# sglang-npu/DeepGEMM_Ascend

Measured on AMD Instinct MI355X. Metric: fp8 TFLOPS + % MFMA peak, 4096^3 block-scaled GEMM; grouped-GEMM tok/s at 1/2/4/8 GPU, higher is better.
Workload: dtype bf16

## Files before the change

deepgemm_ascend_amd/csrc/dga_launch_menu_n.hip:

```cpp
#include <atomic>
#include <cstdlib>
#include "dga_fp8_menu_impl.hpp"
#include "gemm_fp8_bf16x_dsk_kernel.hpp"
namespace dga {

static constexpr int kDskExtraHalfBlocks = 2;

int bx_dsk_splits(int64_t tiles, int kb, int want, int cus)
{
    if (tiles <= 0 || tiles > cus) return 0;
    int s = want > 0 ? want : 1;
    if (s > DskCfg::MAX_S) s = DskCfg::MAX_S;
    if (s > cus / tiles) s = static_cast<int>(cus / tiles);
    if (s > kb / 4) s = kb / 4;
    return s;
}

size_t bx_dsk_workspace_bytes(int64_t tiles, int splits)
{
    if (splits <= 1) return 0;
    return static_cast<size_t>(tiles) * (splits - 1) * (DskCfg::SLOT_FLOATS * 4 + 8) + 256;
}

template <bool KTAIL, bool IMG = true, int OUT = 0>
static int launch_bx_dsk_one(const GemmParams &p, const StreamKArgs &sk, unsigned grid, hipStream_t stream)
{
    constexpr int kLds = IMG ? DskCfg::IMG_LDS_BYTES : DskCfg::LDS_BYTES;
    return launch_kernel<gemm_fp8_bf16x_dsk_kernel<KTAIL, IMG, OUT>>(grid, DskCfg::NT, kLds, stream, p, sk);
}

int launch_bf16x_dsk(const GemmParams &p, int splits, void *ws, size_t ws_bytes, hipStream_t stream, Out out)
{
    if (out == Out::F32Rows) return DGA_E_TILING;
    if (p.groups != 1 || p.masked_m || p.m_indices || p.row_index || p.splitk > 1 || p.tail_sub || p.stamps || p.launch_tiles) return DGA_E_TILING;
    const int cus = coresident_workgroups(stream);
    if (cus <= 0) return DGA_E_TILING;
    GemmParams q = p;
    q.tiles_m = (p.m + DskCfg::BM - 1) / DskCfg::BM;
    q.tiles_n = (p.n + DskCfg::BN - 1) / DskCfg::BN;
    const int64_t tiles = static_cast<int64_t>(q.tiles_m) * q.tiles_n;
    const int s = bx_dsk_splits(tiles, p.kb_n, splits, cus);
    if (s < 1) return DGA_E_TILING;
    q.splitk = s;
    StreamKArgs sk{};
    if (s > 1) {
        const size_t slots = static_cast<size_t>(tiles) * (s - 1);
        if (!ws || ws_bytes < slots * (DskCfg::SLOT_FLOATS * 4 + 8) || (reinterpret_cast<uintptr_t>(ws) & 15)) return DGA_E_TILING;
        sk.partials = static_cast<float *>(ws);
        sk.flags = reinterpret_cast<unsigned long long *>(sk.partials + slots * DskCfg::SLOT_FLOATS);
        static std::atomic<unsigned long long> launches{0};
        const unsigned long long e = launches.fetch_add(1) + 1;
        sk.epoch = (e * 0x9E3779B97F4A7C15ull) | 1ull;
    }
    if (s > 1) {
        int extra = kDskExtraHalfBlocks;
#ifdef DGA_DSK_KNOBS
        if (const char *e = std::getenv("DGA_DSK_EXTRA")) extra = std::atoi(e);
#endif
        for (; extra > 0; --extra) {
            const int wo = (2 * p.kb_n - 2 * extra) / (2 * s), wa = wo + extra;
            if (wo < 4 || wa > 255 || wo > 255) continue;
            const int64_t W = 2 * wa + static_cast<int64_t>(2 * s - 2) * wo;
            auto cut = [&](int i) { return static_cast<int>((static_cast<int64_t>(p.kb_n) * (i <= 2 ? i * wa : 2 * wa + (i - 2) * wo)) / W); };
            bool ok = true;
            for (int i = 0; i < 2 * s && ok; ++i) ok = cut(i + 1) - cut(i) >= 2;
            if (ok) { q.tail_sub = wa | (wo << 8); break; }
        }
    }
#ifdef DGA_DSK_KNOBS
    if (const char *e = std::getenv("DGA_DSK_KNOB")) q.tail_begin = std::atoi(e);
#endif
    const unsigned grid = static_cast<unsigned>(tiles * s);
#ifdef DGA_DSK_KNOBS
    if (q.tail_begin & 64)
        return (p.k % 128) ? launch_bx_dsk_one<true, false>(q, sk, grid, stream) : launch_bx_dsk_one<false, false>(q, sk, grid, stream);
#endif
    if (out == Out::F32) return (p.k % 128) ? launch_bx_dsk_one<true, true, 1>(q, sk, grid, stream) : launch_bx_dsk_one<false, true, 1>(q, sk, grid, stream);
    return (p.k % 128) ? launch_bx_dsk_one<true>(q, sk, grid, stream) : launch_bx_dsk_one<false>(q, sk, grid, stream);
}

}
```

deepgemm_ascend_amd/csrc/gemm_fp8_bf16x_dsk_kernel.hpp:

```cpp
#pragma once
#include "gemm_fp8_kernel.hpp"
#include "gemm_fp8_streamk_kernel.hpp"

namespace dga {

struct DskCfg {
    static constexpr int BM = 64, BN = 128, GT = 256, NT = 512, TN = 2;
    static constexpr int A_BYTES = BM * 128, B_BYTES = BN * 128, SC_BYTES = GT * 4;
    static constexpr int STAGE_BYTES = A_BYTES + B_BYTES + SC_BYTES, RING_BYTES = 3 * STAGE_BYTES, LDS_BYTES = 2 * RING_BYTES;
    static constexpr int IMG_BYTES = BM * 128 * 2, IMG_GROUP_BYTES = 2 * STAGE_BYTES + IMG_BYTES, IMG_LDS_BYTES = 2 * IMG_GROUP_BYTES;
    static constexpr int A_ITERS = 2, B_ITERS = 4, NL = A_ITERS + B_ITERS + 1;
    static constexpr int SLOT_FLOATS = BM * BN;
    static constexpr int MAX_S = 8;
};

template <bool KTAIL, bool IMG = true, int OUT = 0>
__global__ void __launch_bounds__(512) __attribute__((amdgpu_waves_per_eu(2, 2)))
gemm_fp8_bf16x_dsk_kernel(const GemmParams p, const StreamKArgs sk)
{
    typedef DskCfg C;
    constexpr int BM = C::BM, BN = C::BN, GT = C::GT, TN = C::TN, NL = C::NL, LAGT = 2, RING = 4;
    typedef __bf16 v8bf __attribute__((ext_vector_type(8)));
    extern __shared__ __attribute__((aligned(16))) uint8_t smem[];

    const int tid = threadIdx.x, lane = tid & 63, gtid = tid & (GT - 1);
    const int wave = __builtin_amdgcn_readfirstlane(tid >> 6);
    const int h = wave >> 2, gw = wave & 3;
    const int li = lane & 15, kg = lane >> 4;
    const int KB = p.kb_n, S = p.splitk;

    int v = blockIdx.x;
    if (p.xcd_remap) v = xcd_chunk_first(gridDim.x, v & 7) + (v >> 3);
    const int tm = v % p.tiles_m, rest = v / p.tiles_m, s = rest % S, tn = rest / S;
    const int tile = tn * p.tiles_m + tm;
    const int M = p.m, m0 = tm * BM, n0 = tn * BN;
    const int wa = p.tail_sub > 0 ? (p.tail_sub & 0xFF) : 1, wo = p.tail_sub > 0 ? (p.tail_sub >> 8) : 1;
    const int W = 2 * wa + (2 * S - 2) * wo;
    auto cut = [&](int i) { return (int)(((int64_t)KB * (i <= 2 ? i * wa : 2 * wa + (i - 2) * wo)) / W); };
    const int i0 = 2 * s + h, io = 2 * s + (1 - h);
    const int kb0 = cut(i0), kb1 = cut(i0 + 1);
    const int nblk = kb1 - kb0;
    const int nblk_o = cut(io + 1) - cut(io);
    const int nmax = max(nblk, nblk_o);

    uint8_t *const ring = smem + h * (IMG ? C::IMG_GROUP_BYTES : C::RING_BYTES);
    const uint32_t lds0 = (uint32_t)(uintptr_t)(lptr_t)ring;
    constexpr uint32_t kOutOfRange = 0x80000000u;
    const int a_col = ((gtid & 7) ^ swz_a(gtid >> 3)) * 16;
    const int b_col = ((gtid & 7) ^ swz_b(gtid >> 3)) * 16;
    uint32_t a_voff[C::A_ITERS], b_voff[C::B_ITERS];
#pragma unroll
    for (int it = 0; it < C::A_ITERS; ++it) {
        const int row = (it * GT + gtid) >> 3;
        a_voff[it] = row < M - m0 ? (uint32_t)row * (uint32_t)p.lda + a_col : kOutOfRange;
    }
#pragma unroll
    for (int it = 0; it < C::B_ITERS; ++it) {
        const int row = (it * GT + gtid) >> 3;
        b_voff[it] = (uint32_t)min(row, p.n - 1 - n0) * (uint32_t)p.ldb + b_col;
    }
    const v4i a_rsrc = make_rsrc(p.a + (int64_t)m0 * p.lda, (int64_t)(M - m0) * p.lda);
    const v4i b_rsrc = make_rsrc(p.b + (int64_t)n0 * p.ldb, (int64_t)(p.n - n0) * p.ldb);
    const float *const sc_src = gtid < BM ? p.sfa + (int64_t)min(m0 + gtid, M - 1) * p.sfa_ld
                                          : p.sfb + (int64_t)min(n0 / 128, p.nb_n - 1) * p.kb_n;
    auto refill = [&](int idx, int stage, int kb) {
#ifdef DGA_DSK_KNOBS
        if (p.tail_begin & 8) return;
#endif
        const uint32_t sa = lds0 + stage * C::STAGE_BYTES + gw * 1024;
        const int k0 = kb * 128;
        const bool live = kb < kb1;
        if (idx < C::A_ITERS) {
            uint32_t voff = live ? a_voff[idx] : kOutOfRange;
            if constexpr (KTAIL) voff = (k0 + a_col < p.k) ? voff : kOutOfRange;
            dma16(voff, a_rsrc, (uint32_t)k0, sa + idx * GT * 16);
        } else if (idx < C::A_ITERS + C::B_ITERS) {
            const int it = idx - C::A_ITERS;
            uint32_t voff = live ? b_voff[it] : kOutOfRange;
            if constexpr (KTAIL) voff = (k0 + b_col < p.k) ? voff : kOutOfRange;
            dma16(voff, b_rsrc, (uint32_t)k0, sa + C::A_BYTES + it * GT * 16);
        } else {
            dma4(sc_src + (live ? kb : kb1 - 1), lds0 + stage * C::STAGE_BYTES + C::A_BYTES + C::B_BYTES + gw * 256);
        }
    };

    const int a_off0 = li * 128 + ((kg ^ swz_a(li)) * 16);
    const int a_off1 = li * 128 + (((kg + 4) ^ swz_a(li)) * 16);
    const int b_row = gw * (BN / 4) + 8 * (li >> 2) + (li & 3);
    const int b_off0 = C::A_BYTES + b_row * 128 + ((kg ^ swz_b(b_row)) * 16);
    const int b_off1 = C::A_BYTES + b_row * 128 + (((kg + 4) ^ swz_b(b_row)) * 16);
    const int sa_off = C::A_BYTES + C::B_BYTES + li * 4;
    const int sb_off = C::A_BYTES + C::B_BYTES + BM * 4;

    v4f acc[4][TN];
    v4f part[RING];
    v4i afx[2][4], bfx[TN][4];
    v4i braw[TN][2], araw[2][2];
    float s_cur[4], s_old[4];
#pragma unroll
    for (int i = 0; i < 4; ++i)
#pragma unroll
        for (int j = 0; j < TN; ++j) acc[i][j] = v4f{0.f, 0.f, 0.f, 0.f};

#pragma unroll
    for (int d = 0; d < (IMG ? 2 : 3); ++d)
#pragma unroll
        for (int idx = 0; idx < NL; ++idx) refill(idx, d, kb0 + d);

    auto run = [&](auto Lc) __attribute__((always_inline)) {
        constexpr int L = decltype(Lc)::value;
        constexpr int TILES = L * TN, GAPS = 4 * TILES, SP = L;
        static_assert(TILES % RING == 0 && 1 + (NL - 1) * SP < GAPS, "the ring of partial tiles; the refill fits a block");
#pragma unroll
        for (int i = 0; i < RING; ++i) part[i] = v4f{0.f, 0.f, 0.f, 0.f};
#pragma unroll
        for (int i = 0; i < L; ++i) s_old[i] = 0.f;
        int cur = 0;
        for (int it = 0; it < nmax; ++it) {
            if (it == 0) wait_vmcnt<2 * NL>();
            else wait_vmcnt<NL>();
            __builtin_amdgcn_s_barrier();
            asm volatile("" ::: "memory");
#ifdef DGA_DSK_KNOBS
            if ((p.tail_begin & 4) && it < nblk) {
                if (it > 0) for (int idx = 0; idx < NL; ++idx) refill(idx, cur >= 1 ? cur - 1 : 2, kb0 + it + 2);
            } else
#endif
            if (it < nblk) {
                const int fill = cur >= 1 ? cur - 1 : 2, kbf = kb0 + it + 2;
                const uint8_t *sc = ring + cur * C::STAGE_BYTES;
#ifdef DGA_DSK_KNOBS
                if ((p.tail_begin & 32) && it > 0)
                    for (int idx = 0; idx < NL; ++idx) refill(idx, fill, kbf);
#endif
                araw[0][0] = *(const v4i *)(sc + a_off0);
                araw[0][1] = *(const v4i *)(sc + a_off1);
                braw[0][0] = *(const v4i *)(sc + b_off0);
                braw[0][1] = *(const v4i *)(sc + b_off1);
                braw[1][0] = *(const v4i *)(sc + b_off0 + 512);
                braw[1][1] = *(const v4i *)(sc + b_off1 + 512);
                araw[1][0] = *(const v4i *)(sc + a_off0 + 2048);
                araw[1][1] = *(const v4i *)(sc + a_off1 + 2048);
                const float sfb0 = *(const float *)(sc + sb_off);
                float sa[L];
#pragma unroll
                for (int i = 0; i < L; ++i) sa[i] = *(const float *)(sc + sa_off + i * 64);
                __builtin_amdgcn_sched_barrier(0);
#pragma unroll
                for (int c = 0; c < 16; ++c) bx_convert(braw[0], bfx[0], c);
#pragma unroll
                for (int c = 0; c < 16; ++c) bx_convert(araw[0], afx[0], c);
                if constexpr (L > 2) {
                    araw[0][0] = *(const v4i *)(sc + a_off0 + 2 * 2048);
                    araw[0][1] = *(const v4i *)(sc + a_off1 + 2 * 2048);
                }
#pragma unroll
                for (int c = 0; c < 16; ++c) bx_convert(braw[1], bfx[1], c);
#pragma unroll
                for (int i = 0; i < L; ++i) s_cur[i] = sa[i] * sfb0;
                __builtin_amdgcn_sched_barrier(0);
#pragma unroll
                for (int u = 0; u < GAPS; ++u) {
                    const int t = u >> 2, q = u & 3, mt = t / TN, nt = t % TN, g8 = u % (4 * TN);
                    part[t % RING] = __builtin_amdgcn_mfma_f32_16x16x32_bf16(
                        __builtin_bit_cast(v8bf, bfx[nt][q]), __builtin_bit_cast(v8bf, afx[mt & 1][q]),
                        q == 0 ? v4f{0.f, 0.f, 0.f, 0.f} : part[t % RING], 0, 0, 0);
                    __builtin_amdgcn_sched_barrier(0);
#ifdef DGA_DSK_KNOBS
                    if (!(p.tail_begin & 32))
#endif
                    if (u >= 1 && (u - 1) % SP == 0 && (u - 1) / SP < NL && it > 0) refill((u - 1) / SP, fill, kbf);
                    if (mt + 1 < L) {
#pragma unroll
                        for (int c = 2 * g8; c < 2 * g8 + 2; ++c) bx_convert(araw[(mt + 1) & 1], afx[(mt + 1) & 1], c);
                        if (g8 == 4 * TN - 1 && mt + 3 < L) {
                            araw[(mt + 1) & 1][0] = *(const v4i *)(sc + a_off0 + (mt + 3) * 2048);
                            araw[(mt + 1) & 1][1] = *(const v4i *)(sc + a_off1 + (mt + 3) * 2048);
                        }
                    }
                    {
                        const int j = t >= LAGT ? t - LAGT : TILES + t - LAGT, jm = j / TN, jn = j % TN;
                        const float sv = t >= LAGT ? s_cur[jm] : s_old[jm];
                        acc[jm][jn][q] = __builtin_fmaf(part[j % RING][q], sv, acc[jm][jn][q]);
                    }
                    __builtin_amdgcn_sched_barrier(0);
                }
#pragma unroll
                for (int i = 0; i < L; ++i) s_old[i] = s_cur[i];
            }
            cur = cur == 2 ? 0 : cur + 1;
        }
#pragma unroll
        for (int t = 0; t < LAGT; ++t) {
            const int j = TILES + t - LAGT, jm = j / TN, jn = j % TN;
#pragma unroll
            for (int q = 0; q < 4; ++q) acc[jm][jn][q] = __builtin_fmaf(part[j % RING][q], s_old[jm], acc[jm][jn][q]);
        }
    };
    auto run_img = [&](auto Lc) __attribute__((always_inline)) {
        constexpr int L = decltype(Lc)::value;
        constexpr int TILES = L * TN, GAPS = 4 * TILES, SP = L;
        static_assert(TILES % RING == 0 && 1 + (NL - 1) * SP < GAPS, "the ring of partial tiles; the refill fits a block");
        uint8_t *const img = ring + 2 * C::STAGE_BYTES;
#pragma unroll
        for (int i = 0; i < RING; ++i) part[i] = v4f{0.f, 0.f, 0.f, 0.f};
#pragma unroll
        for (int i = 0; i < L; ++i) s_old[i] = 0.f;
        int cur = 0;
        for (int it = 0; it < nmax; ++it) {
            wait_vmcnt<NL>();
            __builtin_amdgcn_s_barrier();
            asm volatile("" ::: "memory");
            const bool live = it < nblk;
            const uint8_t *sc = ring + cur * C::STAGE_BYTES;
            if (live) {
                if (gw < L) {
                    araw[0][0] = *(const v4i *)(sc + a_off0 + gw * 2048);
                    araw[0][1] = *(const v4i *)(sc + a_off1 + gw * 2048);
                }
                braw[0][0] = *(const v4i *)(sc + b_off0);
                braw[0][1] = *(const v4i *)(sc + b_off1);
                braw[1][0] = *(const v4i *)(sc + b_off0 + 512);
                braw[1][1] = *(const v4i *)(sc + b_off1 + 512);
                const float sfb0 = *(const float *)(sc + sb_off);
                float sa[L];
#pragma unroll
                for (int i = 0; i < L; ++i) sa[i] = *(const float *)(sc + sa_off + i * 64);
                if (gw < L) {
#pragma unroll
                    for (int c = 0; c < 16; ++c) bx_convert(araw[0], afx[0], c);
#pragma unroll
                    for (int q = 0; q < 4; ++q) *(v4i *)(img + ((gw * 4 + q) * 64 + lane) * 16) = afx[0][q];
                }
#pragma unroll
                for (int c = 0; c < 16; ++c) bx_convert(braw[0], bfx[0], c);
#pragma unroll
                for (int c = 0; c < 16; ++c) bx_convert(braw[1], bfx[1], c);
#pragma unroll
                for (int i = 0; i < L; ++i) s_cur[i] = sa[i] * sfb0;
            }
            asm volatile("s_waitcnt lgkmcnt(0)" ::: "memory");
            __builtin_amdgcn_s_barrier();
            asm volatile("" ::: "memory");
            if (live) {
                const int kbf = kb0 + it + 2;
#pragma unroll
                for (int q = 0; q < 4; ++q) afx[0][q] = *(const v4i *)(img + (q * 64 + lane) * 16);
                __builtin_amdgcn_sched_barrier(0);
#pragma unroll
                for (int u = 0; u < GAPS; ++u) {
                    const int t = u >> 2, q = u & 3, mt = t / TN, nt = t % TN;
                    part[t % RING] = __builtin_amdgcn_mfma_f32_16x16x32_bf16(
                        __builtin_bit_cast(v8bf, bfx[nt][q]), __builtin_bit_cast(v8bf, afx[mt & 1][q]),
                        q == 0 ? v4f{0.f, 0.f, 0.f, 0.f} : part[t % RING], 0, 0, 0);
                    __builtin_amdgcn_sched_barrier(0);
                    if (u >= 1 && (u - 1) % SP == 0 && (u - 1) / SP < NL) refill((u - 1) / SP, cur, kbf);
                    if (nt == 0 && q == 0 && mt + 1 < L) {
#pragma unroll
                        for (int qq = 0; qq < 4; ++qq) afx[(mt + 1) & 1][qq] = *(const v4i *)(img + (((mt + 1) * 4 + qq) * 64 + lane) * 16);
                    }
                    {
                        const int j = t >= LAGT ? t - LAGT : TILES + t - LAGT, jm = j / TN, jn = j % TN;
                        const float sv = t >= LAGT ? s_cur[jm] : s_old[jm];
                        acc[jm][jn][q] = __builtin_fmaf(part[j % RING][q], sv, acc[jm][jn][q]);
                    }
                    __builtin_amdgcn_sched_barrier(0);
                }
#pragma unroll
                for (int i = 0; i < L; ++i) s_old[i] = s_cur[i];
            }
            cur ^= 1;
        }
#pragma unroll
        for (int t = 0; t < LAGT; ++t) {
            const int j = TILES + t - LAGT, jm = j / TN, jn = j % TN;
#pragma unroll
            for (int q = 0; q < 4; ++q) acc[jm][jn][q] = __builtin_fmaf(part[j % RING][q], s_old[jm], acc[jm][jn][q]);
        }
    };
    if constexpr (IMG) {
        if (M - m0 <= 32) run_img(std::integral_constant<int, 2>{});
        else run_img(std::integral_constant<int, 4>{});
    } else {
        if (M - m0 <= 32) run(std::integral_constant<int, 2>{});
        else run(std::integral_constant<int, 4>{});
    }

    wait_vmcnt<0>();
    __builtin_amdgcn_s_barrier();
    asm volatile("" ::: "memory");
    v4f *const X = reinterpret_cast<v4f *>(smem);
    if (h == 1) {
#pragma unroll
        for (int ti = 0; ti < 8; ++ti) X[(gw * 8 + ti) * 64 + lane] = acc[ti >> 1][ti & 1];
    }
    __syncthreads();
    if (h == 0) {
#pragma unroll
        for (int ti = 0; ti < 8; ++ti) {
            const v4f o = X[(gw * 8 + ti) * 64 + lane];
            v4f &a = acc[ti >> 1][ti & 1];
            a.x += o.x; a.y += o.y; a.z += o.z; a.w += o.w;
        }
    }
    uint16_t *const Cout = p.out;
    const bool vec_ok = ((p.ldc & 7) == 0) && ((((uintptr_t)Cout) & 15) == 0);
    auto store_row = [&](int m, int n, const v4f &lo, const v4f &hi) {
        if (m >= M) return;
        if constexpr (OUT == 1) {
            float *const Cf = reinterpret_cast<float *>(p.out);
            const v4f v[2] = {lo, hi};
            store_row_f32<8>(Cf + (int64_t)m * p.ldc, p.c_in ? p.c_in + (int64_t)m * p.ldc : nullptr, n, p.n,
                             f32_rows_vec(Cf, p.c_in, p.ldc), 0, v);
            return;
        }
        uint16_t *crow = Cout + (int64_t)m * p.ldc;
        const v2bf h0 = __builtin_convertvector(v2f{lo.x, lo.y}, v2bf);
        const v2bf h1 = __builtin_convertvector(v2f{lo.z, lo.w}, v2bf);
        const v2bf h2 = __builtin_convertvector(v2f{hi.x, hi.y}, v2bf);
        const v2bf h3 = __builtin_convertvector(v2f{hi.z, hi.w}, v2bf);
        const v4i pk = v4i{__builtin_bit_cast(int, h0), __builtin_bit_cast(int, h1), __builtin_bit_cast(int, h2), __builtin_bit_cast(int, h3)};
        if (vec_ok && n + 8 <= p.n) {
            *(v4i *)(crow + n) = pk;
        } else {
            const uint16_t *e = (const uint16_t *)&pk;
#pragma unroll
            for (int q = 0; q < 8; ++q)
                if (n + q < p.n) crow[n + q] = e[q];
        }
    };
    if (S == 1) {
        if (h == 0) {
#pragma unroll
            for (int mt = 0; mt < 4; ++mt) store_row(m0 + 16 * mt + li, n0 + gw * (BN / 4) + 8 * kg, acc[mt][0], acc[mt][1]);
        }
        return;
    }
#ifdef DGA_DSK_KNOBS
    const int knob = p.tail_begin;
    if ((knob & 1) && s > 0) return;
#endif
    if (s > 0) {
        const int slot = tile * (S - 1) + (s - 1);
        if (h == 0) {
            float *dst = sk.partials + (int64_t)slot * C::SLOT_FLOATS + (gw * 8 * 64 + lane) * 4;
#pragma unroll
            for (int ti = 0; ti < 8; ++ti) {
                asm volatile("global_store_dwordx4 %0, %1, off sc0 sc1" :: "v"(dst), "v"(acc[ti >> 1][ti & 1]) : "memory");
                dst += 64 * 4;
                asm volatile("" : "+v"(dst));
            }
        }
        wait_vmcnt<0>();
        __builtin_amdgcn_s_barrier();
        asm volatile("" ::: "memory");
        if (tid == 0) __hip_atomic_store(sk.flags + slot, sk.epoch, __ATOMIC_RELAXED, __HIP_MEMORY_SCOPE_AGENT);
        return;
    }
    if (h == 0) {
#pragma unroll
        for (int ti = 0; ti < 8; ++ti) X[(gw * 8 + ti) * 64 + lane] = acc[ti >> 1][ti & 1];
    }
    const int e0 = (gw * 8 + 4 * h) * 64 + lane;
    v4f w[C::MAX_S - 1][4];
    __syncthreads();
#pragma unroll
    for (int j = 0; j < C::MAX_S - 1; ++j) {
        if (j < S - 1) {
#ifdef DGA_DSK_KNOBS
            if (!(knob & 3))
#endif
            if (tid == 0)
                while (__hip_atomic_load(sk.flags + tile * (S - 1) + j, __ATOMIC_RELAXED, __HIP_MEMORY_SCOPE_AGENT) != sk.epoch) __builtin_amdgcn_s_sleep(2);
            __builtin_amdgcn_s_barrier();
            asm volatile("" ::: "memory");
            if (wave != 0) {
                const float *src = sk.partials + (int64_t)(tile * (S - 1) + j) * C::SLOT_FLOATS + e0 * 4;
#pragma unroll
                for (int e = 0; e < 4; ++e) {
                    asm volatile("global_load_dwordx4 %0, %1, off sc0 sc1" : "=v"(w[j][e]) : "v"(src) : "memory");
                    src += 64 * 4;
                    asm volatile("" : "+v"(src));
                }
            }
        }
    }
    if (wave == 0) {
#pragma unroll
        for (int j = 0; j < C::MAX_S - 1; ++j) {
            if (j < S - 1) {
                const float *src = sk.partials + (int64_t)(tile * (S - 1) + j) * C::SLOT_FLOATS + e0 * 4;
#pragma unroll
                for (int e = 0; e < 4; ++e) {
                    asm volatile("global_load_dwordx4 %0, %1, off sc0 sc1" : "=v"(w[j][e]) : "v"(src) : "memory");
                    src += 64 * 4;
                    asm volatile("" : "+v"(src));
                }
            }
        }
    }
    if (tid == 0)
        for (int j = 0; j < S - 1; ++j) __hip_atomic_store(sk.flags + tile * (S - 1) + j, 0ull, __ATOMIC_RELAXED, __HIP_MEMORY_SCOPE_AGENT);
    v4f sum[4];
#pragma unroll
    for (int e = 0; e < 4; ++e) sum[e] = X[e0 + 64 * e];
    wait_vmcnt<0>();
#pragma unroll
    for (int j = 0; j < C::MAX_S - 1; ++j) {
        if (j < S - 1) {
#pragma unroll
            for (int e = 0; e < 4; ++e) {
                asm volatile("" : "+v"(w[j][e]));
                sum[e].x += w[j][e].x; sum[e].y += w[j][e].y; sum[e].z += w[j][e].z; sum[e].w += w[j][e].w;
            }
        }
    }
#pragma unroll
    for (int i = 0; i < 2; ++i) store_row(m0 + 16 * (2 * h + i) + li, n0 + gw * (BN / 4) + 8 * kg, sum[2 * i], sum[2 * i + 1]);
}

}
```

Baseline: 1191.

## Split dual-group reduction across both halves and poll stream-K flags with a wave ballot

The intra-block reduction of the two K-halves now splits work so each half sums and stores half the tile, instead of half 1 writing everything to LDS and half 0 doing all adds and stores. Split-K writers store their half-reduced partials from all waves. The fixer polls all peer flags at once with one wave using a ballot and publishes a bitmask in LDS, so other waves can start loading each partial as soon as it is ready instead of waiting on per-slot barriers. Cut math moves to 32-bit unsigned with a host-side overflow guard, and optional timestamp instrumentation is added behind a compile flag. The LDS spin loops add polling traffic, and the unsigned cut assumes the product stays below 2^31.

```diff
diff --git a/deepgemm_ascend_amd/csrc/dga_launch_menu_n.hip b/deepgemm_ascend_amd/csrc/dga_launch_menu_n.hip
--- a/deepgemm_ascend_amd/csrc/dga_launch_menu_n.hip
+++ b/deepgemm_ascend_amd/csrc/dga_launch_menu_n.hip
@@ -61,6 +61,7 @@
             const int wo = (2 * p.kb_n - 2 * extra) / (2 * s), wa = wo + extra;
             if (wo < 4 || wa > 255 || wo > 255) continue;
             const int64_t W = 2 * wa + static_cast<int64_t>(2 * s - 2) * wo;
+            if (p.kb_n * W > 0x7fffffff) continue;
             auto cut = [&](int i) { return static_cast<int>((static_cast<int64_t>(p.kb_n) * (i <= 2 ? i * wa : 2 * wa + (i - 2) * wo)) / W); };
             bool ok = true;
             for (int i = 0; i < 2 * s && ok; ++i) ok = cut(i + 1) - cut(i) >= 2;
@@ -69,6 +70,9 @@
     }
 #ifdef DGA_DSK_KNOBS
     if (const char *e = std::getenv("DGA_DSK_KNOB")) q.tail_begin = std::atoi(e);
+#endif
+#ifdef DGA_DSK_STAMPS
+    if (const char *e = std::getenv("DGA_DSK_STAMPS_BUF")) q.stamps = reinterpret_cast<unsigned long long *>(std::strtoull(e, nullptr, 0));
 #endif
     const unsigned grid = static_cast<unsigned>(tiles * s);
 #ifdef DGA_DSK_KNOBS
@@ -79,4 +83,11 @@
     return (p.k % 128) ? launch_bx_dsk_one<true>(q, sk, grid, stream) : launch_bx_dsk_one<false>(q, sk, grid, stream);
 }
 
+#ifdef DGA_DSK_STAMPS
+extern "C" int dga_dsk_diag_empty_launch(unsigned grid, void *stream)
+{
+    return launch_kernel<dsk_empty_kernel>(grid, DskCfg::NT, DskCfg::IMG_LDS_BYTES, static_cast<hipStream_t>(stream), static_cast<int *>(nullptr));
 }
+#endif
+
+}
diff --git a/deepgemm_ascend_amd/csrc/gemm_fp8_bf16x_dsk_kernel.hpp b/deepgemm_ascend_amd/csrc/gemm_fp8_bf16x_dsk_kernel.hpp
--- a/deepgemm_ascend_amd/csrc/gemm_fp8_bf16x_dsk_kernel.hpp
+++ b/deepgemm_ascend_amd/csrc/gemm_fp8_bf16x_dsk_kernel.hpp
@@ -14,6 +14,21 @@
     static constexpr int MAX_S = 8;
 };
 
+#ifdef DGA_DSK_STAMPS
+__device__ inline unsigned long long dsk_stamp_pick(const unsigned long long (&st)[16], int lane)
+{
+    unsigned long long v = 0;
+#pragma unroll
+    for (int i = 0; i < 16; ++i) v = lane == i ? st[i] : v;
+    return v;
+}
+__global__ void __launch_bounds__(512) dsk_empty_kernel(int *sink)
+{
+    extern __shared__ __attribute__((aligned(16))) uint8_t smem_e[];
+    if (sink) sink[threadIdx.x] = smem_e[threadIdx.x];
+}
+#endif
+
 template <bool KTAIL, bool IMG = true, int OUT = 0>
 __global__ void __launch_bounds__(512) __attribute__((amdgpu_waves_per_eu(2, 2)))
 gemm_fp8_bf16x_dsk_kernel(const GemmParams p, const StreamKArgs sk)
@@ -28,20 +43,42 @@
     const int h = wave >> 2, gw = wave & 3;
     const int li = lane & 15, kg = lane >> 4;
     const int KB = p.kb_n, S = p.splitk;
+#ifdef DGA_DSK_STAMPS
+    unsigned long long st[16] = {};
+#define DSK_STAMP(i) asm volatile("s_memtime %0\n\ts_waitcnt lgkmcnt(0)" : "=s"(st[i])::"memory")
+#define DSK_FLUSH()                                                                                                             \
+    do {                                                                                                                        \
+        asm volatile("s_memrealtime %0\n\ts_waitcnt lgkmcnt(0)" : "=s"(st[11])::"memory");                                      \
+        if (p.stamps && lane < 16) p.stamps[((size_t)blockIdx.x * 8 + wave) * 16 + lane] = dsk_stamp_pick(st, lane);            \
+    } while (0)
+    asm volatile("s_memtime %0\n\ts_memrealtime %1\n\ts_waitcnt lgkmcnt(0)" : "=s"(st[0]), "=s"(st[10])::"memory");
+    asm volatile("" ::"s"(KB), "s"(S));
+    DSK_STAMP(14);
+#else
+#define DSK_STAMP(i) do { } while (0)
+#define DSK_FLUSH() do { } while (0)
+#endif
 
     int v = blockIdx.x;
-    if (p.xcd_remap) v = xcd_chunk_first(gridDim.x, v & 7) + (v >> 3);
+    if (p.xcd_remap) v = xcd_chunk_first(p.tiles_m * p.tiles_n * S, v & 7) + (v >> 3);
     const int tm = v % p.tiles_m, rest = v / p.tiles_m, s = rest % S, tn = rest / S;
     const int tile = tn * p.tiles_m + tm;
     const int M = p.m, m0 = tm * BM, n0 = tn * BN;
+#ifdef DGA_DSK_STAMPS
+    st[13] = (unsigned)s | ((unsigned)S << 8) | ((unsigned long long)tile << 16);
+#endif
     const int wa = p.tail_sub > 0 ? (p.tail_sub & 0xFF) : 1, wo = p.tail_sub > 0 ? (p.tail_sub >> 8) : 1;
-    const int W = 2 * wa + (2 * S - 2) * wo;
-    auto cut = [&](int i) { return (int)(((int64_t)KB * (i <= 2 ? i * wa : 2 * wa + (i - 2) * wo)) / W); };
-    const int i0 = 2 * s + h, io = 2 * s + (1 - h);
-    const int kb0 = cut(i0), kb1 = cut(i0 + 1);
+    const uint32_t W = 2 * wa + (2 * S - 2) * wo;
+    auto cut = [&](int i) { return (int)(((uint32_t)KB * (uint32_t)(i <= 2 ? i * wa : 2 * wa + (i - 2) * wo)) / W); };
+    const int c0 = cut(2 * s), c1 = cut(2 * s + 1), c2 = cut(2 * s + 2);
+    const int kb0 = h ? c1 : c0, kb1 = h ? c2 : c1;
     const int nblk = kb1 - kb0;
-    const int nblk_o = cut(io + 1) - cut(io);
+    const int nblk_o = h ? c1 - c0 : c2 - c1;
     const int nmax = max(nblk, nblk_o);
+#ifdef DGA_DSK_STAMPS
+    asm volatile("" ::"s"(nmax), "s"(kb0));
+    DSK_STAMP(15);
+#endif
 
     uint8_t *const ring = smem + h * (IMG ? C::IMG_GROUP_BYTES : C::RING_BYTES);
     const uint32_t lds0 = (uint32_t)(uintptr_t)(lptr_t)ring;
@@ -105,7 +142,10 @@
 #pragma unroll
     for (int d = 0; d < (IMG ? 2 : 3); ++d)
 #pragma unroll
-        for (int idx = 0; idx < NL; ++idx) refill(idx, d, kb0 + d);
+        for (int idx = 0; idx < NL; ++idx) {
+            refill(idx, d, kb0 + d);
+            if (d == 0 && idx == 0) DSK_STAMP(1);
+        }
 
     auto run = [&](auto Lc) __attribute__((always_inline)) {
         constexpr int L = decltype(Lc)::value;
@@ -209,8 +249,10 @@
         int cur = 0;
         for (int it = 0; it < nmax; ++it) {
             wait_vmcnt<NL>();
+            if (it == 0) DSK_STAMP(2);
             __builtin_amdgcn_s_barrier();
             asm volatile("" ::: "memory");
+            if (it == 0) DSK_STAMP(3);
             const bool live = it < nblk;
             const uint8_t *sc = ring + cur * C::STAGE_BYTES;
             if (live) {
@@ -286,23 +328,38 @@
         else run(std::integral_constant<int, 4>{});
     }
 
+    DSK_STAMP(4);
     wait_vmcnt<0>();
     __builtin_amdgcn_s_barrier();
     asm volatile("" ::: "memory");
     v4f *const X = reinterpret_cast<v4f *>(smem);
-    if (h == 1) {
-#pragma unroll
-        for (int ti = 0; ti < 8; ++ti) X[(gw * 8 + ti) * 64 + lane] = acc[ti >> 1][ti & 1];
+    const int e0 = (gw * 8 + 4 * h) * 64 + lane;
+    const int x0 = (gw * 8 + 4 * (1 - h)) * 64 + lane;
+    unsigned *const seen_lds = reinterpret_cast<unsigned *>(X + 8 * 4 * 64);
+    if (tid == 0) __hip_atomic_store(seen_lds, 0u, __ATOMIC_RELAXED, __HIP_MEMORY_SCOPE_WORKGROUP);
+    v4f sum[4];
+    if (h == 0) {
+#pragma unroll
+        for (int e = 0; e < 4; ++e) X[x0 + 64 * e] = acc[2 + (e >> 1)][e & 1];
+    } else {
+#pragma unroll
+        for (int e = 0; e < 4; ++e) X[x0 + 64 * e] = acc[e >> 1][e & 1];
     }
     __syncthreads();
     if (h == 0) {
 #pragma unroll
-        for (int ti = 0; ti < 8; ++ti) {
-            const v4f o = X[(gw * 8 + ti) * 64 + lane];
-            v4f &a = acc[ti >> 1][ti & 1];
-            a.x += o.x; a.y += o.y; a.z += o.z; a.w += o.w;
-        }
-    }
+        for (int e = 0; e < 4; ++e) {
+            const v4f a = acc[e >> 1][e & 1], o = X[e0 + 64 * e];
+            sum[e] = v4f{a.x + o.x, a.y + o.y, a.z + o.z, a.w + o.w};
+        }
+    } else {
+#pragma unroll
+        for (int e = 0; e < 4; ++e) {
+            const v4f a = X[e0 + 64 * e], o = acc[2 + (e >> 1)][e & 1];
+            sum[e] = v4f{a.x + o.x, a.y + o.y, a.z + o.z, a.w + o.w};
+        }
+    }
+    DSK_STAMP(5);
     uint16_t *const Cout = p.out;
     const bool vec_ok = ((p.ldc & 7) == 0) && ((((uintptr_t)Cout) & 15) == 0);
     auto store_row = [&](int m, int n, const v4f &lo, const v4f &hi) {
@@ -330,10 +387,10 @@
         }
     };
     if (S == 1) {
-        if (h == 0) {
-#pragma unroll
-            for (int mt = 0; mt < 4; ++mt) store_row(m0 + 16 * mt + li, n0 + gw * (BN / 4) + 8 * kg, acc[mt][0], acc[mt][1]);
-        }
+#pragma unroll
+        for (int i = 0; i < 2; ++i) store_row(m0 + 16 * (2 * h + i) + li, n0 + gw * (BN / 4) + 8 * kg, sum[2 * i], sum[2 * i + 1]);
+        DSK_STAMP(8);
+        DSK_FLUSH();
         return;
     }
 #ifdef DGA_DSK_KNOBS
@@ -342,69 +399,71 @@
 #endif
     if (s > 0) {
         const int slot = tile * (S - 1) + (s - 1);
-        if (h == 0) {
-            float *dst = sk.partials + (int64_t)slot * C::SLOT_FLOATS + (gw * 8 * 64 + lane) * 4;
-#pragma unroll
-            for (int ti = 0; ti < 8; ++ti) {
-                asm volatile("global_store_dwordx4 %0, %1, off sc0 sc1" :: "v"(dst), "v"(acc[ti >> 1][ti & 1]) : "memory");
-                dst += 64 * 4;
-                asm volatile("" : "+v"(dst));
-            }
+        float *dst = sk.partials + (int64_t)slot * C::SLOT_FLOATS + e0 * 4;
+#pragma unroll
+        for (int e = 0; e < 4; ++e) {
+            asm volatile("global_store_dwordx4 %0, %1, off sc0 sc1" :: "v"(dst), "v"(sum[e]) : "memory");
+            dst += 64 * 4;
+            asm volatile("" : "+v"(dst));
         }
         wait_vmcnt<0>();
+        DSK_STAMP(6);
         __builtin_amdgcn_s_barrier();
         asm volatile("" ::: "memory");
         if (tid == 0) __hip_atomic_store(sk.flags + slot, sk.epoch, __ATOMIC_RELAXED, __HIP_MEMORY_SCOPE_AGENT);
+        DSK_STAMP(7);
+        DSK_FLUSH();
         return;
     }
-    if (h == 0) {
-#pragma unroll
-        for (int ti = 0; ti < 8; ++ti) X[(gw * 8 + ti) * 64 + lane] = acc[ti >> 1][ti & 1];
-    }
-    const int e0 = (gw * 8 + 4 * h) * 64 + lane;
     v4f w[C::MAX_S - 1][4];
-    __syncthreads();
+    const unsigned all = (1u << (S - 1)) - 1;
+    unsigned seen = 0;
+#ifdef DGA_DSK_KNOBS
+    if (knob & 3) {
+        seen = all;
+        if (tid == 0) __hip_atomic_store(seen_lds, seen, __ATOMIC_RELAXED, __HIP_MEMORY_SCOPE_WORKGROUP);
+    }
+#endif
 #pragma unroll
     for (int j = 0; j < C::MAX_S - 1; ++j) {
         if (j < S - 1) {
-#ifdef DGA_DSK_KNOBS
-            if (!(knob & 3))
-#endif
-            if (tid == 0)
-                while (__hip_atomic_load(sk.flags + tile * (S - 1) + j, __ATOMIC_RELAXED, __HIP_MEMORY_SCOPE_AGENT) != sk.epoch) __builtin_amdgcn_s_sleep(2);
-            __builtin_amdgcn_s_barrier();
+            if (wave == 0) {
+                while ((seen & all) != all) {
+                    bool up = false;
+                    if (lane < S - 1)
+                        up = __hip_atomic_load(sk.flags + tile * (S - 1) + lane, __ATOMIC_RELAXED, __HIP_MEMORY_SCOPE_AGENT) == sk.epoch;
+                    seen = (unsigned)__builtin_amdgcn_ballot_w64(up);
+                    if (lane == 0) __hip_atomic_store(seen_lds, seen, __ATOMIC_RELAXED, __HIP_MEMORY_SCOPE_WORKGROUP);
+#ifdef DGA_DSK_STAMPS
+                    if (!st[9]) { DSK_STAMP(9); st[12] = seen; }
+#endif
+                    if ((seen & all) != all) __builtin_amdgcn_s_sleep(2);
+                }
+            } else {
+                while (!((seen >> j) & 1)) {
+                    seen = __builtin_amdgcn_readfirstlane(__hip_atomic_load(seen_lds, __ATOMIC_RELAXED, __HIP_MEMORY_SCOPE_WORKGROUP));
+                    if (!((seen >> j) & 1)) __builtin_amdgcn_s_sleep(1);
+                }
+#ifdef DGA_DSK_STAMPS
+                if (j == 0) DSK_STAMP(9);
+#endif
+            }
             asm volatile("" ::: "memory");
-            if (wave != 0) {
-                const float *src = sk.partials + (int64_t)(tile * (S - 1) + j) * C::SLOT_FLOATS + e0 * 4;
-#pragma unroll
-                for (int e = 0; e < 4; ++e) {
-                    asm volatile("global_load_dwordx4 %0, %1, off sc0 sc1" : "=v"(w[j][e]) : "v"(src) : "memory");
-                    src += 64 * 4;
-                    asm volatile("" : "+v"(src));
-                }
-            }
-        }
-    }
-    if (wave == 0) {
-#pragma unroll
-        for (int j = 0; j < C::MAX_S - 1; ++j) {
-            if (j < S - 1) {
-                const float *src = sk.partials + (int64_t)(tile * (S - 1) + j) * C::SLOT_FLOATS + e0 * 4;
-#pragma unroll
-                for (int e = 0; e < 4; ++e) {
-                    asm volatile("global_load_dwordx4 %0, %1, off sc0 sc1" : "=v"(w[j][e]) : "v"(src) : "memory");
-                    src += 64 * 4;
-                    asm volatile("" : "+v"(src));
-                }
-            }
-        }
-    }
-    if (tid == 0)
-        for (int j = 0; j < S - 1; ++j) __hip_atomic_store(sk.flags + tile * (S - 1) + j, 0ull, __ATOMIC_RELAXED, __HIP_MEMORY_SCOPE_AGENT);
-    v4f sum[4];
-#pragma unroll
-    for (int e = 0; e < 4; ++e) sum[e] = X[e0 + 64 * e];
+            const float *src = sk.partials + (int64_t)(tile * (S - 1) + j) * C::SLOT_FLOATS + e0 * 4;
+#pragma unroll
+            for (int e = 0; e < 4; ++e) {
+                asm volatile("global_load_dwordx4 %0, %1, off sc0 sc1" : "=v"(w[j][e]) : "v"(src) : "memory");
+                src += 64 * 4;
+                asm volatile("" : "+v"(src));
+            }
+        }
+    }
+    DSK_STAMP(6);
+    __builtin_amdgcn_s_barrier();
+    asm volatile("" ::: "memory");
+    if (tid < S - 1) __hip_atomic_store(sk.flags + tile * (S - 1) + tid, 0ull, __ATOMIC_RELAXED, __HIP_MEMORY_SCOPE_AGENT);
     wait_vmcnt<0>();
+    DSK_STAMP(7);
 #pragma unroll
     for (int j = 0; j < C::MAX_S - 1; ++j) {
         if (j < S - 1) {
@@ -417,6 +476,10 @@
     }
 #pragma unroll
     for (int i = 0; i < 2; ++i) store_row(m0 + 16 * (2 * h + i) + li, n0 + gw * (BN / 4) + 8 * kg, sum[2 * i], sum[2 * i + 1]);
+    DSK_STAMP(8);
+    DSK_FLUSH();
 }
+#undef DSK_STAMP
+#undef DSK_FLUSH
 
 }
```

After: 1192 (median of 2 runs). Within noise of the previous version (+0.2%).
